# ouyangjiahong/representation-disentanglement

Measured on AMD Instinct MI355X. Metric: MR slices/sec (train step, recon+adv+latent losses), higher is better.
Workload: dtype f32

## Files before the change

include/mrdis.h:

```cpp
#ifndef MRDIS_H
#define MRDIS_H

#include <stddef.h>
#include <stdint.h>

#ifdef __cplusplus
extern "C" {
#endif

#define MRDIS_OK            0
#define MRDIS_EINVAL       -1
#define MRDIS_EUNSUPPORTED -2
#define MRDIS_EWORKSPACE   -3
#define MRDIS_ELAUNCH      -4
#define MRDIS_EALIGN       -5

#define MRDIS_MAX_TAPS 16

#define MRDIS_EPI_NONE   0
#define MRDIS_EPI_LRELU  1

const char* mrdis_strerror(int code);
int mrdis_version(void);

// ... 48 lines not shown
size_t mrdis_wino_u_job_bytes(void);
int mrdis_wino_u_format(int R, int S, int spadeC);
long long mrdis_wino_u_image_floats(int R, int S, int spadeC);
long long mrdis_wino_u_image_floats_fmt(int R, int S, int spadeC, int fmt);
int mrdis_wino_u_job_blocks(int R, int S, int spadeC);
int mrdis_wino_u_jobs(const void* jobs, int njobs, int total_blocks, void* stream);

size_t mrdis_s6_filter_image_bytes(int taps, int Cred, int Cout);
int mrdis_s6_filter_image(const float* w, int taps, int Cred, int Cout, void* image, size_t image_bytes, void* stream);

int mrdis_conv2d_bwd_data(const void* dy, int lddy, const float* w_tkc, const void* w_bf16_tck,
                          void* dx, int lddx, int N, int H, int W, int Ci, int Co,
                          int kh, int kw, int stride, int pad, int dtype, const float* w_wino , int w_wino_fmt, void* stream);

int mrdis_cast_bf16(const float* src, void* dst_bf16, long long n, void* stream);
int mrdis_cast_view(const void* src, int ld_src, int src_dtype, int C_src, void* dst, int ld_dst, int dst_dtype, int C_dst,
                    long long P, void* stream);

int mrdis_copy_bytes(const void* src, void* dst, long long nbytes, void* stream);
int mrdis_stream_fill(float* dst, long long n_floats, float value, void* stream);

int mrdis_instnorm_stats(const void* z, int ldz, float* save_mean, float* save_rstd, void* workspace, size_t workspace_bytes,
                         int N, long long HW, int C, float eps, int dtype, void* stream);
int mrdis_conv2d_fwd_spade(const void* x, int ldx, const float* w_tck, const void* w_bf16_tkc, const float* bias, const void* z, int ldz,
                           const float* mean, const float* rstd, void* mix, int ldmix, void* gamma, int ldg,
                           int N, int H, int W, int Ci, int C, int dtype, const float* w_wino , int w_wino_fmt , void* stream);

size_t mrdis_conv2d_bwd_weight_workspace(int N, int H, int W, int Ci, int Co,
                                         int kh, int kw, int stride, int pad);
int mrdis_conv2d_bwd_weight(const void* x, int ldx, const void* dy, int lddy,
                            float* dw_tck, float* dbias, void* workspace, size_t workspace_bytes,
                            int N, int H, int W, int Ci, int Co,
                            int kh, int kw, int stride, int pad, int accumulate_bias, int dtype, void* stream);

int mrdis_lrelu_bwd(const void* dy, int lddy, const void* y, int ldy, void* dx, int lddx,
                    long long P, int C, float slope, int dtype, void* stream);

size_t mrdis_norm_workspace(int groups, long long P, int C);
int mrdis_bn_train_fwd(const void* x, int ldx, void* y, int ldy, const float* gamma,
                       const float* beta, float* running_mean, float* running_var,
                       float* save_mean, float* save_rstd, void* workspace, size_t workspace_bytes,
                       long long P, int C, float eps, float momentum, int groups, int dtype, void* stream);
int mrdis_bn_eval_fwd(const void* x, int ldx, void* y, int ldy, const float* gamma, const float* beta,
                      const float* running_mean, const float* running_var, long long P, int C, float eps, int dtype, void* stream);
int mrdis_bn_train_bwd(const void* dy, int lddy, const void* x, int ldx, const float* gamma,
                       const float* save_mean, const float* save_rstd, void* dx, int lddx,
                       float* dgamma, float* dbeta, float* acc_dgamma, float* acc_dbeta,
                       void* workspace, size_t workspace_bytes, long long P, int C, int groups, int dtype, void* stream);

int mrdis_instnorm_spade_fwd(const void* z, int ldz, const void* gamma, int ldg,
                             const void* beta, int ldb, void* out, int ldo,
                             float* save_mean, float* save_rstd, void* workspace, size_t workspace_bytes,
                             int N, long long HW, int C, float eps, int dtype, void* stream);
size_t mrdis_instnorm_spade_bwd_workspace(int N, long long HW, int C);
int mrdis_instnorm_spade_bwd(const void* dout, int lddo, const void* z, int ldz,
                             const void* gamma, int ldg, const float* save_mean, const float* save_rstd,
                             void* dz, int lddz, void* dgamma, int lddg, void* dbeta, int lddb,
                             void* workspace, size_t workspace_bytes,
                             int N, long long HW, int C, int dtype, void* stream);
size_t mrdis_instnorm_spade_bwd_up2_workspace(int N, int Hi, int Wi, int C, int dtype);
int mrdis_instnorm_spade_bwd_up2(const void* dout, int lddo, const void* z, int ldz,
                                 const void* gamma, int ldg, const float* save_mean, const float* save_rstd,
                                 void* dx, int lddx, void* dgamma, int lddg, void* dbeta, int lddb,
                                 void* workspace, size_t workspace_bytes,
                                 int N, int Hi, int Wi, int C, const void* xlo, int ldxlo, int dtype, void* stream);

// ... 160 lines not shown
```

representation-disentanglement_amd/csrc/mrdis_common.h:

```cpp
#pragma once
#include <hip/hip_runtime.h>
#include <stdint.h>
#include "../../include/mrdis.h"
#include "mrdis_device.h"

#define MRDIS_CHECK_LAUNCH()                                     \
    do {                                                         \
        hipError_t e_ = hipGetLastError();                       \
        if (e_ != hipSuccess) return MRDIS_ELAUNCH;              \
    } while (0)

#define MRDIS_OPTIONS(X) \
    X(WINO, "wino", "MRDIS_WINO", 0, 1)  \
    X(NT_MB, "nt_mb", "MRDIS_NT_MB", 0, 128)  \
    X(WINO_PIPE, "wino_pipe", "MRDIS_WINO_PIPE", 0, 1)  \
    X(WINO_U, "wino_u", "MRDIS_WINO_U", 0, 1)  \
    X(WINO4, "wino4", "MRDIS_WINO4", 0, 1)  \
    X(WINO4R, "wino4r", "MRDIS_WINO4R", 0, 1)  \
    X(BCONV4, "bconv4", "MRDIS_BCONV4", 0, 1)  \
    X(SPLIT6, "split6", "MRDIS_SPLIT6", 0, 1)  \
    X(NO16, "debug_no16", "MRDIS_DEBUG_NO16", 1, 0) \
    X(NOTHIN, "debug_nothin", "MRDIS_DEBUG_NOTHIN", 1, 0) \
    X(NOC4, "debug_noc4", "MRDIS_DEBUG_NOC4", 1, 0) \
    X(NODMA, "debug_nodma", "MRDIS_DEBUG_NODMA", 1, 0) \
    X(NO16_3D, "debug_no16_3d", "MRDIS_DEBUG_NO16_3D", 1, 0) \
    X(BILGEN, "debug_bilgen", "MRDIS_DEBUG_BILGEN", 1, 0) \
    X(NOW16, "debug_now16", "MRDIS_DEBUG_NOW16", 1, 0) \
    X(NOPACK, "debug_nopack", "MRDIS_DEBUG_NOPACK", 1, 0)  \
    X(MODE, "debug_mode", "MRDIS_DEBUG_MODE", 0, -1) \
    X(BN, "debug_bn", "MRDIS_DEBUG_BN", 0, -1) \
    X(KC, "debug_kc", "MRDIS_DEBUG_KC", 0, -1) \
    X(BM, "debug_bm", "MRDIS_DEBUG_BM", 0, -1) \
    X(C4_TW, "debug_c4_tw", "MRDIS_DEBUG_C4_TW", 0, -1) \
    X(WGSPLIT, "debug_wgsplit", "MRDIS_DEBUG_WGSPLIT", 0, -1) \
    X(BN3, "debug_bn3", "MRDIS_DEBUG_BN3", 0, -1) \
    X(KC3, "debug_kc3", "MRDIS_DEBUG_KC3", 0, -1) \
    X(C4_GRID, "c4_grid", "MRDIS_C4_GRID", 0, 0)  \
    X(C4_BLOCKS, "debug_c4_blocks", "MRDIS_DEBUG_C4_BLOCKS", 0, -1)  \
    X(ZS_GRID, "zsearch_grid", "MRDIS_ZSEARCH_GRID", 0, 0)  \
    X(VOLGEN, "debug_volgen", "MRDIS_DEBUG_VOLGEN", 1, 0)
#define MRDIS_X_OPT_ID(id, name, env, is_flag, dflt) MRDIS_OPT_##id,
enum { MRDIS_OPTIONS(MRDIS_X_OPT_ID) MRDIS_OPT_COUNT };
long long mrdis_opt(int id);
void mrdis_opt_note(int id, long long value);

#define MRDIS_COUNTERS(X) \
    X(WINO, "wino") X(WINO_SPADE, "wino_spade") X(WINO2, "wino2") X(WINO2_SPADE, "wino2_spade") X(WINO4, "wino4") X(WINO4_SPADE, "wino4_spade") X(WINO4N, "wino4n") \
    X(WINO4R, "wino4r") X(WINO_WGRAD, "wino_wgrad") X(WINO_WGRAD2, "wino_wgrad2") X(WINO4_WGRAD, "wino4_wgrad") X(BCONV3, "bconv3") X(BCONV3_SPADE, "bconv3_spade") \
    X(BCONV4, "bconv4") X(BCONV4_SPADE, "bconv4_spade") X(SPLIT6_C4, "split6_c4") X(SPLIT6_C16, "split6_c16") X(SPLIT6_WGRAD16, "split6_wgrad16") X(SPLIT6_CO4, "split6_co4") \
    X(SPLIT6_C3D, "split6_c3d") X(SPLIT6_W3D, "split6_w3d") X(SPLIT6_TAP, "split6_tap") X(ZSEARCH, "zsearch") \
    X(CONV2SRC, "conv2src") X(ANA_ACT, "ana_act")  \
    X(KL, "kl") X(AVGPOOL, "avgpool")  \
    X(CHATT, "chatt") X(SYMDIFF, "symdiff") X(RGATE, "rgate")  \
    X(DIRECT3D, "direct3d") X(C3D16, "c3d16") X(WGRAD3D, "wgrad3d") X(WGRAD3D16, "wgrad3d16") X(WINO_WGRAD3D, "wino_wgrad3d")  \
    X(VOLGATHER, "volgather")  \
    X(LOSS3D, "loss3d") X(SEGCOUNTS, "segcounts")  \
    X(SEGACCUM, "segaccum") X(SEGLABELS, "seglabels")  \
    X(SYNTHACCUM, "synthaccum") X(SYNTHFINISH, "synthfinish")  \
    X(FUSE, "fuse")  \
    X(REGSURF, "regsurf") X(EDT, "edt") X(SURFHIST, "surfhist")  \
    X(STAT_VEC, "stat_vec") X(STAT_SCALAR, "stat_scalar") X(STAT_INTERP, "stat_interp")  \
    X(SPADE_UP2_ONEPASS, "spade_up2_onepass") X(SPADE_UP2_TWOPASS, "spade_up2_twopass")  \
    X(BIL_FWD_X2, "bil_fwd_x2") X(BIL_FWD_GENERAL, "bil_fwd_general")  \
    X(BIL_BWD_X2, "bil_bwd_x2") X(BIL_BWD_TIGHT3, "bil_bwd_tight3") X(BIL_BWD_TIGHT5, "bil_bwd_tight5") X(BIL_BWD_GENERAL, "bil_bwd_general")  \
    X(ELEM_V1, "elem_v1")  \
    X(ALL, "all")
#define MRDIS_X_CNT_ID(id, name) MRDIS_CNT_##id,
enum { MRDIS_COUNTERS(MRDIS_X_CNT_ID) MRDIS_CNT_COUNT };
void mrdis_count(int id);

void mrdis_note_lds(const char* kernel_expr, size_t bytes);
#define MRDIS_LAUNCH(kernel, grid, block, lds, s, ...) do { mrdis_count(MRDIS_CNT_ALL); if ((size_t)(lds) != 0) mrdis_note_lds(#kernel, (size_t)(lds)); hipLaunchKernelGGL(kernel, grid, block, lds, s, __VA_ARGS__); } while (0)

int mrdis_cu_count();
bool mrdis_lds_optin(const void* kernel, int bytes);
int mrdis_occupancy(const void* kernel, int block, size_t lds);

static inline int mrdis_cdiv(long long a, long long b) { return (int)((a + b - 1) / b); }

__device__ __forceinline__ int mrdis_xcd_remap(int bid, int nblk) {
    const int q = nblk >> 3, r = nblk & 7, xcd = bid & 7;
    const int base = (xcd < r) ? xcd * (q + 1) : r * (q + 1) + (xcd - r) * q;
    return base + (bid >> 3);
}

__device__ __forceinline__ float mrdis_wave_sum(float v) {
#pragma unroll
    for (int o = 32; o > 0; o >>= 1) v += __shfl_down(v, o, 64);
    return v;
}
__device__ __forceinline__ double mrdis_wave_sum_d(double v) {
#pragma unroll
    for (int o = 32; o > 0; o >>= 1) v += __shfl_down(v, o, 64);
    return v;
}

int mrdis_launch_slab_reduce(const float* slab, float* dw, int total, int Co, int nslab, const float* bslab, float* dbias, int accumulate_bias,
// ... 2 lines not shown
```

representation-disentanglement_amd/hip.py:

```python
import collections
import ctypes
import os

import torch

_HERE = os.path.dirname(os.path.abspath(__file__))
LIB_PATH = os.path.join(_HERE, 'csrc', 'libmrdis_hip.so')


class MrdisLibraryError(RuntimeError):
    pass


class MrdisError(RuntimeError):
    pass


_lib = None
_c = ctypes
_P, _I, _L, _F, _Z = _c.c_void_p, _c.c_int, _c.c_longlong, _c.c_float, _c.c_size_t

_SIGS = {
    'mrdis_strerror': (_c.c_char_p, [_I]),
    'mrdis_version': (_I, []),
# ... 2 lines not shown
    'mrdis_launch_count': (_L, [_c.c_char_p]),
    'mrdis_launch_count_reset': (None, []),
    'mrdis_dynamic_lds_table': (_I, [_c.c_char_p, _I]),
    'mrdis_mix_experts_fwd': (_I, [_P, _P, _P, _P, _I, _I, _I, _I, _P]),
    'mrdis_mix_experts_bwd_workspace': (_Z, [_I, _I, _I, _I]),
    'mrdis_mix_experts_bwd': (_I, [_P, _P, _P, _P, _P, _P, _Z, _I, _I, _I, _I, _P]),
    'mrdis_mix_experts_routed_fwd': (_I, [_P, _P, _P, _P, _I, _P, _P, _P, _I, _I, _I, _I, _P]),
    'mrdis_mix_experts_routed_bwd': (_I, [_P, _P, _P, _P, _I, _P, _P, _P, _P, _Z, _I, _I, _I, _I, _P]),
    'mrdis_copy_bytes': (_I, [_P, _P, _L, _P]),
    'mrdis_stream_fill': (_I, [_P, _L, _F, _P]),
    'mrdis_instnorm_stats': (_I, [_P, _I, _P, _P, _P, _Z, _I, _L, _I, _F, _I, _P]),
    'mrdis_conv2d_fwd_spade': (_I, [_P, _I, _P, _P, _P, _P, _I, _P, _P, _P, _I, _P, _I, _I, _I, _I, _I, _I, _I, _P, _I, _P]),
    'mrdis_wino_u_job_bytes': (_Z, []),
    'mrdis_wino_u_format': (_I, [_I, _I, _I]),
    'mrdis_wino_u_image_floats': (_L, [_I, _I, _I]),
    'mrdis_s6_filter_image_bytes': (ctypes.c_size_t, [_I, _I, _I]),
    'mrdis_s6_filter_image': (_I, [_P, _I, _I, _I, _P, ctypes.c_size_t, _P]),
    'mrdis_wino_u_image_floats_fmt': (_L, [_I, _I, _I, _I]),
    'mrdis_wino_u_job_blocks': (_I, [_I, _I, _I]),
    'mrdis_wino_u_jobs': (_I, [_P, _I, _I, _P]),
    'mrdis_mix_experts_routed_multi_fwd': (_I, [_P, _P, _P, _P, _I, _I, _P, _P, _P, _P, _P, _I, _L, _I, _I, _I, _I, _P]),
    'mrdis_mix_experts_routed_multi_bwd_workspace': (_Z, [_I, _I, _I, _I, _I]),
    'mrdis_mix_experts_routed_multi_bwd': (_I, [_P, _P, _P, _P, _I, _I, _P, _P, _P, _I, _I, _P, _Z, _I, _I, _I, _I, _P]),
    'mrdis_mix_job_bytes': (_Z, []),
    'mrdis_mix_job_blocks': (_I, [_I, _I, _I]),
    'mrdis_mix_jobs_fwd': (_I, [_P, _I, _I, _P, _I, _I, _P]),
    'mrdis_mix_jobs_bwd': (_I, [_P, _I, _I, _P, _P, _I, _I, _P]),
    'mrdis_conv2d_fwd': (_I, [_P, _I, _P, _P, _P, _P, _I] + [_I] * 11 + [_P, _I, _P]),
    'mrdis_conv2d_bwd_data': (_I, [_P, _I, _P, _P, _P, _I] + [_I] * 10 + [_P, _I, _P]),
    'mrdis_cast_bf16': (_I, [_P, _P, _L, _P]),
    'mrdis_cast_view': (_I, [_P, _I, _I, _I, _P, _I, _I, _I, _L, _P]),
    'mrdis_conv2d_bwd_weight_workspace': (_Z, [_I] * 9),
    'mrdis_conv2d_bwd_weight': (_I, [_P, _I, _P, _I, _P, _P, _P, _Z] + [_I] * 11 + [_P]),
    'mrdis_lrelu_bwd': (_I, [_P, _I, _P, _I, _P, _I, _L, _I, _F, _I, _P]),
    'mrdis_norm_workspace': (_Z, [_I, _L, _I]),
    'mrdis_bn_train_fwd': (_I, [_P, _I, _P, _I, _P, _P, _P, _P, _P, _P, _P, _Z, _L, _I, _F, _F, _I, _I, _P]),
    'mrdis_bn_eval_fwd': (_I, [_P, _I, _P, _I, _P, _P, _P, _P, _L, _I, _F, _I, _P]),
    'mrdis_bn_train_bwd': (_I, [_P, _I, _P, _I, _P, _P, _P, _P, _I, _P, _P, _P, _P, _P, _Z, _L, _I, _I, _I, _P]),
    'mrdis_instnorm_spade_fwd': (_I, [_P, _I, _P, _I, _P, _I, _P, _I, _P, _P, _P, _Z, _I, _L, _I, _F, _I, _P]),
    'mrdis_instnorm_spade_bwd_workspace': (_Z, [_I, _L, _I]),
    'mrdis_instnorm_spade_bwd': (_I, [_P, _I, _P, _I, _P, _I, _P, _P, _P, _I, _P, _I, _P, _I, _P, _Z, _I, _L, _I, _I, _P]),
    'mrdis_instnorm_spade_bwd_up2_workspace': (_Z, [_I, _I, _I, _I, _I]),
    'mrdis_instnorm_spade_bwd_up2': (_I, [_P, _I, _P, _I, _P, _I, _P, _P, _P, _I, _P, _I, _P, _I, _P, _Z, _I, _I, _I, _I, _P, _I, _I, _P]),
    'mrdis_bilinear_fwd': (_I, [_P, _I, _P, _I] + [_I] * 8 + [_P]),
    'mrdis_bilinear_bwd': (_I, [_P, _I, _P, _I] + [_I] * 8 + [_P]),
    'mrdis_bilinear_up2_stats_workspace': (_Z, [_I, _I, _I]),
    'mrdis_bilinear_up2_stats_applies': (_I, [_I, _I, _I]),
    'mrdis_bilinear_up2_stats_fwd': (_I, [_P, _I, _P, _I, _I, _I, _I, _I, _I, _L, _P, _P, _F, _P, _Z, _I, _P]),
    'mrdis_softmax_mask_drop_fwd': (_I, [_P, _I, _P, _P, _I, _L, _I, _F, _P]),
    'mrdis_softmax_mask_drop_bwd': (_I, [_P, _I, _P, _I, _P, _I, _L, _I, _P]),
    'mrdis_recon_err_workspace': (_Z, [_I, _L, _I]),
    'mrdis_recon_err_fwd': (_I, [_P, _I, _P, _I, _P, _P, _Z, _I, _L, _I, _I, _P]),
    'mrdis_recon_err_bwd': (_I, [_P, _I, _P, _I, _P, _P, _I, _I, _L, _I, _I, _P]),
    'mrdis_recon_metrics_workspace': (_Z, [_I, _I]),
    'mrdis_recon_metrics': (_I, [_P, _I, _P, _I, _P, _P, _Z, _I, _I, _I, _P]),
    'mrdis_slice_gather': (_I, [_P, _P, _P, _P, _I, _P, _P, _I, _I, _I, _I, _I, _I, _P]),
    'mrdis_volume_gather': (_I, [_P, _I, _P, _P, _I, _I, _I, _I, _I, _I, _I, _I, _I, _I, _P]),
    'mrdis_nvnet_loss_workspace': (_Z, [_L, _L]),
    'mrdis_nvnet_loss_fwd': (_I, [_P, _P, _P, _P, _P, _I, _P, _P, _P, _P, _P, _I, _c.c_double, _P, _P, _P, _Z, _P]),
    'mrdis_nvnet_loss_bwd': (_I, [_P, _P, _P, _P, _P, _I, _P, _P, _P, _P, _P, _I, _c.c_double, _P, _P, _P, _P, _P]),
    'mrdis_seg_counts': (_I, [_P, _P, _P, _I, _L, _I, _I, _P]),
    'mrdis_seg_accum': (_I, [_P, _P, _I, _I, _I, _I, _I, _I, _I, _I, _P]),
    'mrdis_seg_label_volume': (_I, [_P, _P, _P, _P, _P, _I, _I, _I, _I, _I, _I, _P]),
    'mrdis_synth_accum': (_I, [_P, _I, _P, _P, _I, _I, _I, _I, _I, _I, _I, _I, _P]),
    'mrdis_synth_finish': (_I, [_P, _P, _P, _I, _I, _I, _F, _P]),
    'mrdis_fuse_present_fwd': (_I, [_P, _P, _I, _P, _I, _P, _I, _I, _L, _I, _P]),
# ... 47 lines not shown
    if _lib is not None:
        return _lib
    path = path or LIB_PATH
    if not os.path.exists(path):
        raise MrdisLibraryError(
            f'{path} not found: build it with `python __graft_entry__.py` / `make -C '
            f'{os.path.dirname(path)}`.  There is no CPU or eager fallback for the hot path.')
    lib = ctypes.CDLL(path)
    for name, (res, args) in _SIGS.items():
        fn = getattr(lib, name)
        fn.restype, fn.argtypes = res, args
    _lib = lib
    return lib


def _chk(rc, what):
    if rc != 0:
        raise MrdisError(f'{what}: {load().mrdis_strerror(rc).decode()} ({rc})')


def set_option(name, value):
    _chk(load().mrdis_set_option(name.encode(), int(value)), f'set_option({name})')


def get_option(name):
    return int(load().mrdis_get_option(name.encode()))


OPTION_NAMES = ('wino', 'nt_mb', 'wino_pipe', 'wino_u', 'wino4', 'wino4r', 'bconv4', 'split6', 'debug_no16', 'debug_nothin', 'debug_noc4', 'debug_nodma',
                'debug_no16_3d', 'debug_bilgen', 'debug_now16', 'debug_nopack', 'debug_mode', 'debug_bn', 'debug_kc', 'debug_bm', 'debug_c4_tw',
                'debug_wgsplit', 'debug_bn3', 'debug_kc3', 'c4_grid', 'debug_c4_blocks', 'zsearch_grid', 'debug_volgen')


def options_snapshot():
    return {n: get_option(n) for n in OPTION_NAMES}


def options_restore(snap):
    for n, v in snap.items():
        if get_option(n) != v:
            set_option(n, v)


KERNEL_FAMILIES = WINO_FAMILIES = ('wino', 'wino_spade', 'wino2', 'wino2_spade', 'wino4', 'wino4_spade', 'wino4n', 'wino4r', 'wino_wgrad', 'wino_wgrad2', 'wino4_wgrad', 'bconv3', 'bconv3_spade', 'bconv4', 'bconv4_spade',
                                   'split6_c4', 'split6_c16', 'split6_wgrad16', 'split6_co4', 'split6_c3d', 'split6_w3d', 'split6_tap',
                                   'all',
                                   'zsearch')
VARIANT_FAMILIES = ('conv2src', 'ana_act')
LATENT_FAMILIES = ('kl', 'avgpool')
OUTDEC_FAMILIES = ('chatt', 'symdiff', 'rgate')
CONV3D_FAMILIES = ('direct3d', 'c3d16', 'wgrad3d', 'wgrad3d16', 'wino_wgrad3d')
DATA_FAMILIES = ('volgather',)
LOSS3D_FAMILIES = ('loss3d', 'segcounts')
SEGVOL_FAMILIES = ('segaccum', 'seglabels')
SYNTH_FAMILIES = ('synthaccum', 'synthfinish')
FUSE_FAMILIES = ('fuse',)
SURFDIST_FAMILIES = ('regsurf', 'edt', 'surfhist')
ELEM_FAMILIES = ('stat_vec', 'stat_scalar', 'stat_interp', 'spade_up2_onepass', 'spade_up2_twopass', 'bil_fwd_x2', 'bil_fwd_general',
                 'bil_bwd_x2', 'bil_bwd_tight3', 'bil_bwd_tight5', 'bil_bwd_general', 'elem_v1')
SYNTH_MAX_SRC = 8
FUSE_MAX_SRC = 8
FUSE_METHODS = ('mean', 'max', 'mean-max-min')
EDT_FAR = 1 << 30
EDT_MAX_SRC = 8
EDT_MAX_EXTENT = 1024
SURF_MAX_REGIONS = 4


def stream_fill(t, value=0.0):
    assert t.dtype == torch.float32 and t.numel() % 4 == 0
    _chk(load().mrdis_stream_fill(t.data_ptr(), t.numel(), float(value), _stream()), 'stream_fill')
    return t


def dynamic_lds():
    import re
    buf = _c.create_string_buffer(16384)
    load().mrdis_dynamic_lds_table(buf, 16384)
    out = {}
    for line in buf.value.decode().splitlines():
        expr, _, b = line.rpartition('=')
        if not expr or not b.isdigit():
            continue
        name = re.sub(r'<.*', '', expr.strip().lstrip('(')).strip()
        out[name] = max(out.get(name, 0), int(b))
    return out


def launch_counts(reset=False, elem=False):
    lib = load()
    fams = WINO_FAMILIES + VARIANT_FAMILIES + LATENT_FAMILIES + OUTDEC_FAMILIES + CONV3D_FAMILIES + DATA_FAMILIES + LOSS3D_FAMILIES + SEGVOL_FAMILIES + SYNTH_FAMILIES + FUSE_FAMILIES + SURFDIST_FAMILIES
    out = {f: int(lib.mrdis_launch_count(f.encode())) for f in fams + (ELEM_FAMILIES if elem else ())}
    if reset:
        lib.mrdis_launch_count_reset()
    return out


class option:

    def __init__(self, name, value):
        self.name, self.value = name, value

    def __enter__(self):
        self.prev = get_option(self.name)
        set_option(self.name, self.value)

    def __exit__(self, *exc):
        set_option(self.name, self.prev)


_DEV_INDEX = None


def _stream():
    global _DEV_INDEX
    if _DEV_INDEX is None:
        _DEV_INDEX = torch.cuda.current_device()
    return torch._C._cuda_getCurrentRawStream(_DEV_INDEX)


def _ptr(t):
    return None if t is None else t.data_ptr()


# ... 447 lines not shown
def conv2d_bwd_weight(x, dy, kh, kw, stride, pad, need_bias=True, bias_sink=None, dtype=DT_F32, may_decline=False, pad16=False):
    lib = load()
    x, ldx = nhwc(x)
    dy, lddy = nhwc(dy)
    N, Ci, H, W = x.shape
    Co = dy.shape[1]
    if pad16:
        assert x.dtype is not dy.dtype and 4 in (Ci, Co), 'pad16: the four-channel mixed-storage kernels only'
    dw = torch.empty((kh * kw, 16 if (pad16 and Ci == 4) else Ci, 16 if (pad16 and Co == 4 and Ci != 4) else Co), dtype=torch.float32, device=x.device)
    db = torch.empty(Co, dtype=torch.float32, device=x.device) if (need_bias and bias_sink is None) else None
    nb = _ws_bytes(lib.mrdis_conv2d_bwd_weight_workspace, N, H, W, Ci, Co, kh, kw, stride, pad)
    if nb == 0:
        raise MrdisError('conv2d_bwd_weight: unsupported geometry')
    ws = _ws(nb, x.device)
    sink = bias_sink if (need_bias and bias_sink is not None) else None
    if x.dtype is not dy.dtype:
        rc = lib.mrdis_conv2d_bwd_weight(_ptr(x), ldx, _ptr(dy), lddy, _ptr(dw), _ptr(sink if sink is not None else db), _ptr(ws), nb,
                                         N, H, W, Ci, Co, kh, kw, stride, pad, 1 if sink is not None else 0, _dt_xy(x, dy) | (DT_DW_PAD16 if pad16 else 0), _stream())
        if rc == -2 and may_decline:
            return None
        _chk(rc, 'conv2d_bwd_weight (mixed storage)')
        return dw, db
    if _dt(x, dy) == DT_BF16:
        rc = lib.mrdis_conv2d_bwd_weight(_ptr(x), ldx, _ptr(dy), lddy, _ptr(dw), _ptr(sink if sink is not None else db), _ptr(ws), nb,
                                         N, H, W, Ci, Co, kh, kw, stride, pad, 1 if sink is not None else 0, DT_BF16, _stream())
        if rc == -2:
            fallbacks['conv2d_bwd_weight_bf16'] += 1
            return conv2d_bwd_weight(cast_view(x, torch.float32), cast_view(dy, torch.float32), kh, kw, stride, pad, need_bias, bias_sink, DT_F32)
        _chk(rc, 'conv2d_bwd_weight')
        return dw, db
    _chk(lib.mrdis_conv2d_bwd_weight(_ptr(x), ldx, _ptr(dy), lddy, _ptr(dw), _ptr(sink if sink is not None else db), _ptr(ws), nb,
                                     N, H, W, Ci, Co, kh, kw, stride, pad, 1 if sink is not None else 0, DT_BF16 if _dt(x, dy) == DT_BF16 else int(dtype), _stream()), 'conv2d_bwd_weight')
    return dw, db


def lrelu_bwd(dy, y, slope=0.2):
    lib = load()
    dy, lddy = nhwc(dy); y, ldy = nhwc(y)
    N, C, H, W = y.shape
    dx = empty_nhwc(N, C, H, W, y.device, y.dtype)
    _chk(lib.mrdis_lrelu_bwd(_ptr(dy), lddy, _ptr(y), ldy, _ptr(dx), C, N * H * W, C, slope, _dt(dy, y), _stream()), 'lrelu_bwd')
    return dx


def bn_train_fwd(x, gamma, beta, running_mean, running_var, eps, momentum, out=None, groups=1):
    lib = load()
    x, ldx = nhwc(x)
    N, C, H, W = x.shape
    assert N % groups == 0
    P = (N // groups) * H * W
    if out is None:
        out = empty_nhwc(N, C, H, W, x.device, x.dtype)
    y, ldy = nhwc(out)
    assert y.data_ptr() == out.data_ptr()
    mean = torch.empty(groups * C, dtype=torch.float32, device=x.device)
    rstd = torch.empty(groups * C, dtype=torch.float32, device=x.device)
    nb = groups * _ws_bytes(lib.mrdis_norm_workspace, 1, P, C)
    ws = _ws(nb, x.device)
    _chk(lib.mrdis_bn_train_fwd(_ptr(x), ldx, _ptr(y), ldy, _ptr(gamma), _ptr(beta), _ptr(running_mean), _ptr(running_var),
                                _ptr(mean), _ptr(rstd), _ptr(ws), nb, P, C, eps, momentum, groups, _dt(x, y), _stream()), 'bn_train_fwd')
    return out, mean, rstd


def bn_eval_fwd(x, gamma, beta, running_mean, running_var, eps):
    lib = load()
    x, ldx = nhwc(x)
# ... 1030 lines not shown
```

representation-disentanglement_amd/ops.py:

```python
import contextlib
import numpy as _np
import os as _os

import torch
from torch.autograd import Function

from . import hip


class _MixExperts(Function):

    @staticmethod
    def forward(ctx, W, r):
        w_tck, w_tkc = hip.mix_experts_fwd(W, r)
        ctx.save_for_backward(W, r)
        ctx.mark_non_differentiable(w_tkc)
        return w_tck, w_tkc

    @staticmethod
    def backward(ctx, g_tck, _g_tkc):
        W, r = ctx.saved_tensors
        dW, dr = hip.mix_experts_bwd(g_tck, W, r)
        return dW, dr

# ... 641 lines not shown
            return y4
        return y if Co_p == Co else hip.cast_view(y, torch.float32, Co)

    @staticmethod
    def backward(ctx, dy):
        G, B, share_x, kh, kw, pad, lrelu, dt, Ci, Co, Ci_p, Co_p, x_dtype, padded, Cif, Cof = ctx.meta
        xin, y = ctx.saved_tensors[0], ctx.saved_tensors[1]
        tkcs = ctx.saved_tensors[2:]
        bias = ctx.bias_param
        dy4 = None
        if ctx.head:
            dy = hip.cast_view(dy, torch.float32)
        elif Co_p != Co:
            if Co == 4 and dy.dtype == torch.float32 and (kh, kw, pad, ctx.stride) == (3, 3, 1, 1) and not lrelu and tkcs[0].shape[1] == 16:
                dy4 = dy
            dy = hip.cast_view(dy, torch.bfloat16, Co_p) if dy4 is None else None
        elif dy.dtype != ctx.ydtype:
            dy = hip.cast_view(dy, ctx.ydtype)
        if lrelu:
            dy = hip.lrelu_bwd(dy, y, 0.2)
        dy_dev = (dy if dy is not None else dy4).device
        pad_box = [dy]

        def dy_pad():
            if pad_box[0] is None:
                pad_box[0] = hip.cast_view(dy4, torch.bfloat16, Co_p)
            return pad_box[0]
        H, W = ctx.xshape
        x32 = ctx.x32
        xdt = torch.bfloat16 if _COMPUTE_DTYPE == hip.DT_BF16 else x_dtype
        if xin is not None:
            xdt = xin.dtype
        need_x = ctx.needs_input_grad[0]
        dxb = None
        dx4 = None
        if need_x and x32 is not None and dy is not None and dy.dtype == torch.bfloat16 and tkcs[0].shape[2] == 16:
            dx4 = hip.empty_nhwc(G * B, 4, H, W, dy_dev, torch.float32)
            for g in range(G):
                if hip.conv2d_bwd_data(dy[g * B:(g + 1) * B], tkcs[g], (H, W), 3, 3, 1, 1, out=dx4[g * B:(g + 1) * B], may_decline=True) is None:
                    dx4 = None
                    break
        if need_x and dx4 is None:
            if ctx.dx_in_gb and not share_x and Ci_p == Ci and xin is not None and xin.dtype == x_dtype:
                gbuf = hip.empty_nhwc(G * B, 2 * Ci, H, W, xin.device, xin.dtype)
                gbuf._mrdis_gb_private = True
                dxb = gbuf[:, Ci:]
            else:
                dxb = hip.empty_nhwc(G * B, Ci_p, H, W, dy_dev, xdt)
        sink = _grad_sink(bias) if (bias is not None and Co_p == Co) else None
        dws, db_total = [], None
        for g in range(G):
            dyg = dy[g * B:(g + 1) * B] if dy is not None else None
            if need_x and dx4 is None:
                if dy4 is None or dxb.dtype != torch.bfloat16 or hip.conv2d_bwd_data(dy4[g * B:(g + 1) * B], tkcs[g], (H, W), 3, 3, 1, 1, out=dxb[g * B:(g + 1) * B],
                                                                                      may_decline=True) is None:
                    if dyg is None:
                        dyg = dy_pad()[g * B:(g + 1) * B]
                    wb_g = ctx.wbs[g] if ctx.wbs[g] is not None else s6_dgrad_image(dyg, tkcs[g], (H, W), kh, kw, ctx.stride)
                    hip.conv2d_bwd_data(dyg, tkcs[g], (H, W), kh, kw, ctx.stride, pad, w_bf16=wb_g, out=dxb[g * B:(g + 1) * B])
            res = None
            if dy4 is not None and x32 is None and xin is not None and xin.dtype == torch.bfloat16 and not _NO_CO4B_WGRAD:
                p16 = Cof == 16 and Cif == xin.shape[1]
                r4 = hip.conv2d_bwd_weight(xin if share_x else xin[g * B:(g + 1) * B], dy4[g * B:(g + 1) * B], 3, 3, 1, 1, need_bias=bias is not None, may_decline=True,
                                           pad16=p16)
                if r4 is not None:
                    dw4, db4 = r4
# ... 1042 lines not shown
```

Measured before the change: 250.6.

## Fuse shared-input 3x3 conv data and weight gradients into one kernel

Adds a fused backward kernel for the 4-channel shared-input 3x3 conv. One wave group computes the data gradient with MFMA plus a rolling row accumulation, while the other computes weight and bias gradients from the same dy rows staged in LDS. Partial results go to per-split slabs and a second kernel reduces them. This removes separate bwd-data and bwd-weight launches and repeated dy reads across groups, at the cost of a complex warp-specialised kernel and a large LDS footprint.

Result: slower. 199.6 (-20.3%).

```diff
diff --git a/include/mrdis.h b/include/mrdis.h
--- a/include/mrdis.h
+++ b/include/mrdis.h
@@ -104,6 +104,12 @@
                             float* dw_tck, float* dbias, void* workspace, size_t workspace_bytes,
                             int N, int H, int W, int Ci, int Co,
                             int kh, int kw, int stride, int pad, int accumulate_bias, int dtype, void* stream);
+
+#define MRDIS_SI_BWD_MAX_G 8
+size_t mrdis_si_bwd_workspace(int G, int B, int H, int W, int C);
+int mrdis_si_bwd(const float* x, int ldx, const void* dy, int lddy, const float* const* w_tkc, float* dx, int lddx, float* const* dw_tck,
+                 float* dbias, void* workspace, size_t workspace_bytes, int G, int B, int H, int W, int C,
+                 int kh, int kw, int stride, int pad, int accumulate_bias, int dtype, void* stream);
 
 int mrdis_lrelu_bwd(const void* dy, int lddy, const void* y, int ldy, void* dx, int lddx,
                     long long P, int C, float slope, int dtype, void* stream);
diff --git a/representation-disentanglement_amd/csrc/mrdis_common.h b/representation-disentanglement_amd/csrc/mrdis_common.h
--- a/representation-disentanglement_amd/csrc/mrdis_common.h
+++ b/representation-disentanglement_amd/csrc/mrdis_common.h
@@ -38,7 +38,8 @@
     X(C4_GRID, "c4_grid", "MRDIS_C4_GRID", 0, 0)  \
     X(C4_BLOCKS, "debug_c4_blocks", "MRDIS_DEBUG_C4_BLOCKS", 0, -1)  \
     X(ZS_GRID, "zsearch_grid", "MRDIS_ZSEARCH_GRID", 0, 0)  \
-    X(VOLGEN, "debug_volgen", "MRDIS_DEBUG_VOLGEN", 1, 0)
+    X(VOLGEN, "debug_volgen", "MRDIS_DEBUG_VOLGEN", 1, 0)  \
+    X(SI_BWD, "si_bwd", "MRDIS_SI_BWD", 0, 1)
 #define MRDIS_X_OPT_ID(id, name, env, is_flag, dflt) MRDIS_OPT_##id,
 enum { MRDIS_OPTIONS(MRDIS_X_OPT_ID) MRDIS_OPT_COUNT };
 long long mrdis_opt(int id);
@@ -63,6 +64,7 @@
     X(SPADE_UP2_ONEPASS, "spade_up2_onepass") X(SPADE_UP2_TWOPASS, "spade_up2_twopass")  \
     X(BIL_FWD_X2, "bil_fwd_x2") X(BIL_FWD_GENERAL, "bil_fwd_general")  \
     X(BIL_BWD_X2, "bil_bwd_x2") X(BIL_BWD_TIGHT3, "bil_bwd_tight3") X(BIL_BWD_TIGHT5, "bil_bwd_tight5") X(BIL_BWD_GENERAL, "bil_bwd_general")  \
+    X(SI_BWD, "si_bwd")  \
     X(ELEM_V1, "elem_v1")  \
     X(ALL, "all")
 #define MRDIS_X_CNT_ID(id, name) MRDIS_CNT_##id,
diff --git a/representation-disentanglement_amd/csrc/mrdis_si_bwd.hip b/representation-disentanglement_amd/csrc/mrdis_si_bwd.hip
--- /dev/null
+++ b/representation-disentanglement_amd/csrc/mrdis_si_bwd.hip
@@ -0,0 +1,349 @@
+#include "mrdis_common.h"
+
+namespace {
+constexpr unsigned SI_OOB = 0xfffffff0u;
+
+struct SiBwdParams {
+    const float* x; const float* dy; float* dx; float* slab; float* bias_slab;
+    const float* w[MRDIS_SI_BWD_MAX_G];
+    int G, B, H, ldx, lddy, lddx;
+    int rowp, R, segs, splits;
+    unsigned x_bytes, dy_bytes;
+};
+}
+
+template <int HALVES, int TPW, bool SPLIT>
+__global__ __launch_bounds__(512) void si_bwd_kernel(const SiBwdParams p) {
+    constexpr int C = 16 * HALVES, KS = C / 4, NG = HALVES / 2, NT = HALVES, MT = 3, DYP = C + 16, W = 64 * TPW, WP = W + 2;
+    extern __shared__ __attribute__((aligned(16))) float smem[];
+    float* zs = smem;
+    float* xs = smem + 9 * WP * 4;
+    float* dys = xs + 4 * p.rowp;
+    const int role = __builtin_amdgcn_readfirstlane((int)threadIdx.x >> 8);
+    const int tid = threadIdx.x & 255, lane = tid & 63, wave = tid >> 6, l16 = lane & 15, kq = lane >> 4;
+    const int split = mrdis_xcd_remap((int)blockIdx.x, (int)gridDim.x);
+    const int n = split / p.segs, r0 = (split - n * p.segs) * p.R, r1 = min(r0 + p.R, p.H);
+    const int nzero = 9 * WP * 4 + 4 * p.rowp;
+    const int nfinal = 2 * MT + (p.bias_slab != nullptr ? 1 : 0);
+
+    for (int g = 0; g < p.G; ++g) {
+        __syncthreads();
+        for (int i = threadIdx.x; i < nzero; i += 512) smem[i] = 0.f;
+        if (role == 0) {
+            const int ng = g * p.B + n;
+            const float* wg = p.w[g];
+            const __amdgpu_buffer_rsrc_t rs_x = mrdis_buffer_rsrc(p.x, p.x_bytes);
+            const __amdgpu_buffer_rsrc_t rs_y = mrdis_buffer_rsrc(p.dy, p.dy_bytes);
+            float a[SPLIT ? 1 : KS][3];
+            bf16x8 ab[SPLIT ? NG : 1][3][3];
+            {
+                const int co = l16 >> 2, tl = l16 & 3;
+#pragma unroll
+                for (int rt = 0; rt < 3; ++rt) {
+                    const int tap = 4 * rt + tl, tf = 8 - tap;
+                    if (SPLIT) {
+#pragma unroll
+                        for (int h = 0; h < NG; ++h)
+#pragma unroll
+                            for (int j = 0; j < 8; ++j) {
+                                const int ch = 32 * h + 16 * (j >> 2) + 4 * kq + (j & 3);
+                                const float wv = tap < 9 ? wg[(tf * C + ch) * 4 + co] : 0.f;
+                                __bf16 hi, mid, lo; mrdis_split3(wv, hi, mid, lo);
+                                ab[h][rt][0][j] = hi; ab[h][rt][1][j] = mid; ab[h][rt][2][j] = lo;
+                            }
+                    } else {
+#pragma unroll
+                        for (int ks = 0; ks < KS; ++ks) {
+                            const int ch = 16 * (ks >> 2) + 4 * kq + (ks & 3);
+                            a[ks][rt] = tap < 9 ? wg[(tf * C + ch) * 4 + co] : 0.f;
+                        }
+                    }
+                }
+            }
+            u32x4 xr[TPW][HALVES];
+            auto load_tile = [&](int t, int r) {
+                const int px = 16 * (wave + 4 * t) + l16;
+                const bool ok = (unsigned)r < (unsigned)p.H && r >= r0 - 1 && r <= r1;
+                const unsigned base = 4u * (unsigned)(((ng * p.H + r) * W + px) * p.lddy + 4 * kq);
+#pragma unroll
+                for (int h = 0; h < HALVES; ++h) xr[t][h] = __builtin_amdgcn_raw_buffer_load_b128(rs_y, (int)(ok ? base + 64u * h : SI_OOB), 0, 0);
+            };
+            auto load_x = [&](int iy) {
+                const bool ok = tid < W && (unsigned)iy < (unsigned)p.H && iy <= r1;
+                return __builtin_amdgcn_raw_buffer_load_b128(rs_x, (int)(ok ? 4u * (unsigned)(((n * p.H + iy) * W + tid) * p.ldx) : SI_OOB), 0, 0);
+            };
+            auto store_x = [&](int iy, u32x4 v) {
+                if (tid < W) *reinterpret_cast<u32x4*>(xs + ((iy + 1) & 3) * p.rowp + (tid + 1) * 4) = v;
+            };
+            float4 runA = make_float4(0.f, 0.f, 0.f, 0.f), runB = runA;
+            auto tap_row = [&](int ty, int pcol) {
+                const float4 z0 = *reinterpret_cast<const float4*>(zs + ((3 * ty + 0) * WP + pcol + 0) * 4);
+                const float4 z1 = *reinterpret_cast<const float4*>(zs + ((3 * ty + 1) * WP + pcol + 1) * 4);
+                const float4 z2 = *reinterpret_cast<const float4*>(zs + ((3 * ty + 2) * WP + pcol + 2) * 4);
+                return make_float4((z0.x + z1.x) + z2.x, (z0.y + z1.y) + z2.y, (z0.z + z1.z) + z2.z, (z0.w + z1.w) + z2.w);
+            };
+
+            u32x4 xq = load_x(r0 - 1);
+#pragma unroll
+            for (int t = 0; t < TPW; ++t) load_tile(t, r0 - 1);
+            __syncthreads();
+            store_x(r0 - 1, xq);
+            xq = load_x(r0);
+            for (int r = r0 - 1; r <= r1; ++r) {
+                float* dyr = dys + (r & 1) * (W * DYP);
+                float4* dxp = reinterpret_cast<float4*>(p.dx + ((long long)(n * p.H + r - 1) * W + tid) * p.lddx);
+                float4 prev = make_float4(0.f, 0.f, 0.f, 0.f);
+                if (g > 0 && tid < W && r - 1 >= r0) prev = *dxp;
+#pragma unroll
+                for (int t = 0; t < TPW; ++t) {
+                    f32x4 za[3] = {f32x4{0.f, 0.f, 0.f, 0.f}, f32x4{0.f, 0.f, 0.f, 0.f}, f32x4{0.f, 0.f, 0.f, 0.f}};
+                    if (SPLIT) {
+#pragma unroll
+                        for (int q = 0; q < NG; ++q) {
+                            const unsigned u[8] = {xr[t][2 * q].x, xr[t][2 * q].y, xr[t][2 * q].z, xr[t][2 * q].w, xr[t][2 * q + 1].x, xr[t][2 * q + 1].y, xr[t][2 * q + 1].z, xr[t][2 * q + 1].w};
+                            bf16x8 xh, xm, xl;
+#pragma unroll
+                            for (int j = 0; j < 8; ++j) mrdis_split3(__uint_as_float(u[j]), xh, xm, xl, j);
+#pragma unroll
+                            for (int rt = 0; rt < 3; ++rt) {
+                                za[rt] = __builtin_amdgcn_mfma_f32_16x16x32_bf16(ab[q][rt][1], xm, za[rt], 0, 0, 0);
+                                za[rt] = __builtin_amdgcn_mfma_f32_16x16x32_bf16(ab[q][rt][0], xl, za[rt], 0, 0, 0);
+                                za[rt] = __builtin_amdgcn_mfma_f32_16x16x32_bf16(ab[q][rt][2], xh, za[rt], 0, 0, 0);
+                            }
+#pragma unroll
+                            for (int rt = 0; rt < 3; ++rt) {
+                                za[rt] = __builtin_amdgcn_mfma_f32_16x16x32_bf16(ab[q][rt][0], xm, za[rt], 0, 0, 0);
+                                za[rt] = __builtin_amdgcn_mfma_f32_16x16x32_bf16(ab[q][rt][1], xh, za[rt], 0, 0, 0);
+                                za[rt] = __builtin_amdgcn_mfma_f32_16x16x32_bf16(ab[q][rt][0], xh, za[rt], 0, 0, 0);
+                            }
+                        }
+                    } else {
+#pragma unroll
+                        for (int h = 0; h < HALVES; ++h) {
+                            const float xv[4] = {__uint_as_float(xr[t][h].x), __uint_as_float(xr[t][h].y), __uint_as_float(xr[t][h].z), __uint_as_float(xr[t][h].w)};
+#pragma unroll
+                            for (int j = 0; j < 4; ++j)
+#pragma unroll
+                                for (int rt = 0; rt < 3; ++rt) za[rt] = __builtin_amdgcn_mfma_f32_16x16x4f32(a[4 * h + j][rt], xv[j], za[rt], 0, 0, 0);
+                        }
+                    }
+                    const int px = 16 * (wave + 4 * t) + l16;
+#pragma unroll
+                    for (int h = 0; h < HALVES; ++h) *reinterpret_cast<u32x4*>(dyr + px * DYP + 16 * h + 4 * kq) = xr[t][h];
+                    load_tile(t, r + 1);
+                    float* zd = zs + (px + 1) * 4 + kq;
+#pragma unroll
+                    for (int rt = 0; rt < 3; ++rt)
+#pragma unroll
+                        for (int q = 0; q < 4; ++q)
+                            if (4 * rt + q < 9) zd[(4 * rt + q) * WP * 4] = za[rt][q];
+                }
+                store_x(r + 1, xq);
+                xq = load_x(r + 2);
+                __syncthreads();
+                if (tid < W) {
+                    const float4 g0 = tap_row(0, tid), g1 = tap_row(1, tid), g2 = tap_row(2, tid);
+                    float4 o = make_float4(runB.x + g2.x, runB.y + g2.y, runB.z + g2.z, runB.w + g2.w);
+                    if (r - 1 >= r0) {
+                        if (g > 0) o = make_float4(prev.x + o.x, prev.y + o.y, prev.z + o.z, prev.w + o.w);
+                        *dxp = o;
+                    }
+                    runB = make_float4(runA.x + g1.x, runA.y + g1.y, runA.z + g1.z, runA.w + g1.w);
+                    runA = g0;
+                }
+                __syncthreads();
+            }
+            for (int i = 0; i < nfinal; ++i) __syncthreads();
+        } else {
+            int acol[MT], aty[MT]; bool aok[MT];
+#pragma unroll
+            for (int mt = 0; mt < MT; ++mt) {
+                const int m = mt * 16 + l16;
+                aok[mt] = m < 36;
+                const int tap = aok[mt] ? m >> 2 : 0, ci = m & 3;
+                aty[mt] = tap / 3;
+                acol[mt] = (tap % 3) * 4 + ci + 4 * kq;
+            }
+            const int boff = kq * DYP + l16;
+            f32x4 acc[MT][NT];
+#pragma unroll
+            for (int mt = 0; mt < MT; ++mt)
+#pragma unroll
+                for (int nt = 0; nt < NT; ++nt) acc[mt][nt] = f32x4{0.f, 0.f, 0.f, 0.f};
+            float bsum[NT];
+#pragma unroll
+            for (int nt = 0; nt < NT; ++nt) bsum[nt] = 0.f;
+            __syncthreads();
+            for (int r = r0 - 1; r <= r1; ++r) {
+                const int rw = r - 1;
+                const bool own = rw >= r0 && rw < r1;
+                const float* dyr = dys + (rw & 1) * (W * DYP);
+                int ao[MT];
+#pragma unroll
+                for (int mt = 0; mt < MT; ++mt) ao[mt] = ((rw + aty[mt]) & 3) * p.rowp + acol[mt];
+                constexpr int nsteps = W >> 4;
+                auto steps = [&](int i0, int i1) {
+                    float bvn[NT], avn[MT];
+                    auto read_ops = [&](int i) {
+                        const int ox0 = 4 * (wave + 4 * i);
+#pragma unroll
+                        for (int nt = 0; nt < NT; ++nt) bvn[nt] = dyr[ox0 * DYP + boff + 16 * nt];
+#pragma unroll
+                        for (int mt = 0; mt < MT; ++mt) avn[mt] = xs[ao[mt] + 4 * ox0];
+                    };
+                    read_ops(i0);
+                    for (int i = i0; i < i1; ++i) {
+                        float bv[NT], av[MT];
+#pragma unroll
+                        for (int nt = 0; nt < NT; ++nt) { bv[nt] = bvn[nt]; bsum[nt] += bv[nt]; }
+#pragma unroll
+                        for (int mt = 0; mt < MT; ++mt) av[mt] = aok[mt] ? avn[mt] : 0.f;
+                        read_ops(i + 1 < i1 ? i + 1 : i);
+#pragma unroll
+                        for (int mt = 0; mt < MT; ++mt)
+#pragma unroll
+                            for (int nt = 0; nt < NT; ++nt) acc[mt][nt] = __builtin_amdgcn_mfma_f32_16x16x4f32(av[mt], bv[nt], acc[mt][nt], 0, 0, 0);
+                    }
+                };
+                if (own) steps(0, nsteps / 2);
+                __syncthreads();
+                if (own) steps(nsteps / 2, nsteps);
+                __syncthreads();
+            }
+            float* red = smem;
+            float* out = p.slab + ((long long)g * p.splits + split) * 36 * C;
+#pragma unroll
+            for (int mt = 0; mt < MT; ++mt) {
+#pragma unroll
+                for (int nt = 0; nt < NT; ++nt)
+#pragma unroll
+                    for (int q = 0; q < 4; ++q) red[(wave * NT + nt) * 256 + (4 * kq + q) * 16 + l16] = acc[mt][nt][q];
+                __syncthreads();
+                for (int e = tid; e < NT * 256; e += 256) {
+                    const int nt = e >> 8, rr = (e >> 4) & 15, cc = e & 15, m = mt * 16 + rr;
+                    const float v = (red[e] + red[NT * 256 + e]) + (red[2 * NT * 256 + e] + red[3 * NT * 256 + e]);
+                    if (m < 36) out[m * C + nt * 16 + cc] = v;
+                }
+                __syncthreads();
+            }
+            if (p.bias_slab != nullptr) {
+#pragma unroll
+                for (int nt = 0; nt < NT; ++nt) {
+                    float b = bsum[nt];
+                    b += __shfl_xor(b, 16, 64);
+                    b += __shfl_xor(b, 32, 64);
+                    if (kq == 0) red[(wave * NT + nt) * 16 + l16] = b;
+                }
+                __syncthreads();
+                if (tid < C) {
+                    const int nt = tid >> 4, cc = tid & 15;
+                    p.bias_slab[((long long)g * p.splits + split) * C + tid] =
+                        (red[nt * 16 + cc] + red[(NT + nt) * 16 + cc]) + (red[(2 * NT + nt) * 16 + cc] + red[(3 * NT + nt) * 16 + cc]);
+                }
+            }
+        }
+    }
+}
+
+struct SiDwPtrs { float* d[MRDIS_SI_BWD_MAX_G]; };
+__global__ __launch_bounds__(1024) void si_bwd_reduce_kernel(const float* __restrict__ slab, const SiDwPtrs dw, int G, int total, int C, int nslab,
+                                                             const float* __restrict__ bslab, float* __restrict__ dbias, int accumulate_bias) {
+    __shared__ float red[32][33];
+    const int g = blockIdx.y;
+    const int nout = total + ((dbias != nullptr && g == 0) ? C : 0);
+    const int i = blockIdx.x * 32 + threadIdx.x, y = threadIdx.y;
+    const float* src = nullptr; long long stride = 0; int cnt = 0;
+    if (i < total) { src = slab + (long long)g * nslab * total + i; stride = total; cnt = nslab; }
+    else if (i < nout) { src = bslab + (i - total); stride = C; cnt = nslab * G; }
+    float s0 = 0.f, s1 = 0.f, s2 = 0.f, s3 = 0.f;
+    if (src != nullptr) {
+        int k = y;
+        for (; k + 96 < cnt; k += 128) {
+            s0 += src[(long long)k * stride]; s1 += src[(long long)(k + 32) * stride];
+            s2 += src[(long long)(k + 64) * stride]; s3 += src[(long long)(k + 96) * stride];
+        }
+        for (; k < cnt; k += 32) s0 += src[(long long)k * stride];
+    }
+    red[y][threadIdx.x] = (s0 + s1) + (s2 + s3);
+    __syncthreads();
+    if (y == 0 && i < nout) {
+        float t = 0.f;
+        for (int k = 0; k < 32; ++k) t += red[k][threadIdx.x];
+        if (i < total) {
+            float* d = dw.d[0];
+#pragma unroll
+            for (int q = 1; q < MRDIS_SI_BWD_MAX_G; ++q) if (q == g) d = dw.d[q];
+            d[i] = t;
+        }
+        else { const int c = i - total; dbias[c] = accumulate_bias ? dbias[c] + t : t; }
+    }
+}
+
+static bool plan_si_bwd(SiBwdParams& p, int G, int B, int H, int W, int C) {
+    if (G < 1 || G > MRDIS_SI_BWD_MAX_G || B < 1 || H < 1) return false;
+    if ((C != 32 && C != 64 && C != 128) || (W != 64 && W != 128 && W != 256)) return false;
+    if ((long long)W * C > 256 * 32) return false;
+    p = SiBwdParams{};
+    p.G = G; p.B = B; p.H = H;
+    int rowp = (W + 2) * 4;
+    while ((rowp & 63) != 12) ++rowp;
+    p.rowp = rowp;
+    int segs = mrdis_cdiv(512, B);
+    if (segs > H / 4) segs = H / 4 > 0 ? H / 4 : 1;
+    p.R = mrdis_cdiv(H, segs); p.segs = mrdis_cdiv(H, p.R);
+    p.splits = B * p.segs;
+    return true;
+}
+
+extern "C" size_t mrdis_si_bwd_workspace(int G, int B, int H, int W, int C) {
+    SiBwdParams p;
+    if (!plan_si_bwd(p, G, B, H, W, C)) return 0;
+    return sizeof(float) * ((size_t)G * p.splits * 36 * C + (size_t)G * p.splits * C) + 256;
+}
+
+extern "C" int mrdis_si_bwd(const float* x, int ldx, const void* dy, int lddy, const float* const* w_tkc, float* dx, int lddx, float* const* dw_tck,
+                            float* dbias, void* workspace, size_t workspace_bytes, int G, int B, int H, int W, int C,
+                            int kh, int kw, int stride, int pad, int accumulate_bias, int dtype, void* stream) {
+    if (dtype != MRDIS_DT_F32 || kh != 3 || kw != 3 || stride != 1 || pad != 1 || mrdis_opt(MRDIS_OPT_SI_BWD) == 0) return MRDIS_EUNSUPPORTED;
+    SiBwdParams p;
+    if (!plan_si_bwd(p, G, B, H, W, C)) return MRDIS_EUNSUPPORTED;
+    if (!x || !dy || !w_tkc || !dx || !dw_tck || !workspace || ldx < 4 || lddy < C || lddx < 4) return MRDIS_EINVAL;
+    if (ldx % 4 != 0 || lddy % 4 != 0 || lddx % 4 != 0 || ((((uintptr_t)x) | ((uintptr_t)dy) | ((uintptr_t)dx) | ((uintptr_t)workspace)) & 15) != 0) return MRDIS_EUNSUPPORTED;
+    const long long npx = (long long)B * H * W;
+    const long long xb = 4LL * ((npx - 1) * ldx + 4), yb = 4LL * ((npx * G - 1) * lddy + C);
+    if (xb >= 0x7fffffffLL || yb >= 0x7fffffffLL || npx * lddx >= 0x7fffffffLL) return MRDIS_EUNSUPPORTED;
+    if (workspace_bytes < mrdis_si_bwd_workspace(G, B, H, W, C)) return MRDIS_EWORKSPACE;
+    for (int g = 0; g < G; ++g) {
+        if (!w_tkc[g] || !dw_tck[g]) return MRDIS_EINVAL;
+        p.w[g] = w_tkc[g];
+    }
+    p.x = x; p.dy = reinterpret_cast<const float*>(dy); p.dx = dx; p.ldx = ldx; p.lddy = lddy; p.lddx = lddx;
+    p.x_bytes = (unsigned)xb; p.dy_bytes = (unsigned)yb;
+    p.slab = reinterpret_cast<float*>(workspace);
+    p.bias_slab = dbias ? p.slab + (size_t)G * p.splits * 36 * C : nullptr;
+    const int NT = C / 16;
+    size_t lds = sizeof(float) * ((size_t)9 * (W + 2) * 4 + (size_t)4 * p.rowp + (size_t)2 * W * (C + 16));
+    const size_t red = sizeof(float) * (size_t)(4 * NT * 256);
+    if (lds < red) lds = red;
+    if (lds > 156 * 1024) return MRDIS_EUNSUPPORTED;
+    hipStream_t s = (hipStream_t)stream;
+    const int sp6 = (int)mrdis_opt(MRDIS_OPT_SPLIT6);
+    const bool split = (sp6 == 1 || sp6 == 3 || sp6 == 4) && C <= 64;
+#define SI_GO(hv, tp, sp) { if (!mrdis_lds_optin((const void*)si_bwd_kernel<hv, tp, sp>, 156 * 1024)) return MRDIS_EUNSUPPORTED; \
+                            MRDIS_LAUNCH((si_bwd_kernel<hv, tp, sp>), dim3(p.splits), dim3(512), lds, s, p); }
+#define SI_LAUNCH(hv, tp) { if (split) SI_GO(hv, tp, true) else SI_GO(hv, tp, false) }
+    const int tpw = W / 64;
+    if (NT == 2) { if (tpw == 4) SI_LAUNCH(2, 4) else if (tpw == 2) SI_LAUNCH(2, 2) else SI_LAUNCH(2, 1) }
+    else if (NT == 4) { if (tpw == 2) SI_LAUNCH(4, 2) else SI_LAUNCH(4, 1) }
+    else SI_GO(8, 1, false)
+#undef SI_LAUNCH
+#undef SI_GO
+    MRDIS_CHECK_LAUNCH();
+    mrdis_count(MRDIS_CNT_SI_BWD);
+    const int total = 36 * C, nout = total + (dbias ? C : 0);
+    SiDwPtrs d;
+    for (int g = 0; g < MRDIS_SI_BWD_MAX_G; ++g) d.d[g] = g < G ? dw_tck[g] : nullptr;
+    MRDIS_LAUNCH(si_bwd_reduce_kernel, dim3(mrdis_cdiv(nout, 32), G), dim3(32, 32), 0, s, p.slab, d, G, total, C, p.splits, p.bias_slab, dbias, accumulate_bias);
+    MRDIS_CHECK_LAUNCH();
+    return MRDIS_OK;
+}
diff --git a/representation-disentanglement_amd/hip.py b/representation-disentanglement_amd/hip.py
--- a/representation-disentanglement_amd/hip.py
+++ b/representation-disentanglement_amd/hip.py
@@ -58,6 +58,8 @@
     'mrdis_cast_view': (_I, [_P, _I, _I, _I, _P, _I, _I, _I, _L, _P]),
     'mrdis_conv2d_bwd_weight_workspace': (_Z, [_I] * 9),
     'mrdis_conv2d_bwd_weight': (_I, [_P, _I, _P, _I, _P, _P, _P, _Z] + [_I] * 11 + [_P]),
+    'mrdis_si_bwd_workspace': (_Z, [_I] * 5),
+    'mrdis_si_bwd': (_I, [_P, _I, _P, _I, _P, _P, _I, _P, _P, _P, _Z] + [_I] * 11 + [_P]),
     'mrdis_lrelu_bwd': (_I, [_P, _I, _P, _I, _P, _I, _L, _I, _F, _I, _P]),
     'mrdis_norm_workspace': (_Z, [_I, _L, _I]),
     'mrdis_bn_train_fwd': (_I, [_P, _I, _P, _I, _P, _P, _P, _P, _P, _P, _P, _Z, _L, _I, _F, _F, _I, _I, _P]),
@@ -171,6 +173,9 @@
                 'debug_wgsplit', 'debug_bn3', 'debug_kc3', 'c4_grid', 'debug_c4_blocks', 'zsearch_grid', 'debug_volgen')
 
 
+SCOPED_OPTION_NAMES = ('si_bwd',)
+
+
 def options_snapshot():
     return {n: get_option(n) for n in OPTION_NAMES}
 
@@ -197,6 +202,8 @@
 SURFDIST_FAMILIES = ('regsurf', 'edt', 'surfhist')
 ELEM_FAMILIES = ('stat_vec', 'stat_scalar', 'stat_interp', 'spade_up2_onepass', 'spade_up2_twopass', 'bil_fwd_x2', 'bil_fwd_general',
                  'bil_bwd_x2', 'bil_bwd_tight3', 'bil_bwd_tight5', 'bil_bwd_general', 'elem_v1')
+SI_BWD_FAMILIES = ('si_bwd',)
+SI_BWD_MAX_G = 8
 SYNTH_MAX_SRC = 8
 FUSE_MAX_SRC = 8
 FUSE_METHODS = ('mean', 'max', 'mean-max-min')
@@ -228,7 +235,7 @@
 
 def launch_counts(reset=False, elem=False):
     lib = load()
-    fams = WINO_FAMILIES + VARIANT_FAMILIES + LATENT_FAMILIES + OUTDEC_FAMILIES + CONV3D_FAMILIES + DATA_FAMILIES + LOSS3D_FAMILIES + SEGVOL_FAMILIES + SYNTH_FAMILIES + FUSE_FAMILIES + SURFDIST_FAMILIES
+    fams = WINO_FAMILIES + VARIANT_FAMILIES + LATENT_FAMILIES + OUTDEC_FAMILIES + CONV3D_FAMILIES + DATA_FAMILIES + LOSS3D_FAMILIES + SEGVOL_FAMILIES + SYNTH_FAMILIES + FUSE_FAMILIES + SURFDIST_FAMILIES + SI_BWD_FAMILIES
     out = {f: int(lib.mrdis_launch_count(f.encode())) for f in fams + (ELEM_FAMILIES if elem else ())}
     if reset:
         lib.mrdis_launch_count_reset()
@@ -742,6 +749,36 @@
     _chk(lib.mrdis_conv2d_bwd_weight(_ptr(x), ldx, _ptr(dy), lddy, _ptr(dw), _ptr(sink if sink is not None else db), _ptr(ws), nb,
                                      N, H, W, Ci, Co, kh, kw, stride, pad, 1 if sink is not None else 0, DT_BF16 if _dt(x, dy) == DT_BF16 else int(dtype), _stream()), 'conv2d_bwd_weight')
     return dw, db
+
+
+def si_bwd(x, dy, w_tkcs, need_bias=True, bias_sink=None, kh=3, kw=3, stride=1, pad=1):
+    lib = load()
+    G = len(w_tkcs)
+    if x.dtype is not torch.float32 or dy.dtype is not torch.float32 or x.dim() != 4 or x.shape[1] != 4 or not 1 <= G <= SI_BWD_MAX_G or dy.shape[0] != G * x.shape[0]:
+        return None
+    x, ldx = nhwc(x)
+    dy, lddy = nhwc(dy)
+    B, _, H, W = x.shape
+    C = dy.shape[1]
+    if tuple(dy.shape[2:]) != (H, W) or any(tuple(w.shape) != (9, C, 4) or w.dtype is not torch.float32 for w in w_tkcs):
+        return None
+    nb = _ws_bytes(lib.mrdis_si_bwd_workspace, G, B, H, W, C)
+    if nb == 0:
+        return None
+    ws = _ws(nb, x.device)
+    ws_t = [w.contiguous() for w in w_tkcs]
+    dx = empty_nhwc(B, 4, H, W, x.device)
+    dws = [torch.empty((9, 4, C), dtype=torch.float32, device=x.device) for _ in range(G)]
+    sink = bias_sink if (need_bias and bias_sink is not None) else None
+    db = torch.empty(C, dtype=torch.float32, device=x.device) if (need_bias and sink is None) else None
+    wp = (_c.c_void_p * G)(*[w.data_ptr() for w in ws_t])
+    dp = (_c.c_void_p * G)(*[d.data_ptr() for d in dws])
+    rc = lib.mrdis_si_bwd(_ptr(x), ldx, _ptr(dy), lddy, wp, _ptr(dx), 4, dp, _ptr(sink if sink is not None else db), _ptr(ws), nb,
+                          G, B, H, W, C, kh, kw, stride, pad, 1 if sink is not None else 0, DT_F32, _stream())
+    if rc == -2:
+        return None
+    _chk(rc, 'si_bwd')
+    return dx, dws, db
 
 
 def lrelu_bwd(dy, y, slope=0.2):
diff --git a/representation-disentanglement_amd/ops.py b/representation-disentanglement_amd/ops.py
--- a/representation-disentanglement_amd/ops.py
+++ b/representation-disentanglement_amd/ops.py
@@ -697,6 +697,15 @@
         if xin is not None:
             xdt = xin.dtype
         need_x = ctx.needs_input_grad[0]
+        if (need_x and share_x and dt == hip.DT_F32 and not ctx.head and (kh, kw, pad, ctx.stride) == (3, 3, 1, 1) and (Ci, Ci_p, Cif) == (4, 4, 4) and Co_p == Co
+                and dy is not None and dy.dtype == torch.float32 and xin is not None and xin.dtype == torch.float32):
+            fused = hip.si_bwd(xin, dy, list(tkcs), need_bias=bias is not None, bias_sink=_grad_sink(bias) if bias is not None else None)
+            if fused is not None:
+                dx, dws_g, db_total = fused
+                dws = []
+                for dw in dws_g:
+                    dws += [dw, None]
+                return (dx, db_total, None, None, None, None, None, None, None, None) + tuple(dws)
         dxb = None
         dx4 = None
         if need_x and x32 is not None and dy is not None and dy.dtype == torch.bfloat16 and tkcs[0].shape[2] == 16:
```
